# andreicuceu/vega

Hardware: AMD Instinct MI355X
Metric: model+chi2 evals/sec (Lya auto+cross) (higher is better)
Workload: dtype f64

## Files before the change

### vega_amd/csrc/vegamx.hip

```cpp
#include "vmx_device.h"
#include "vmx_fit.h"
#include "vmx_ensemble.h"
#include "vmx_nested.h"
#include "vmx_smc.h"

#include <atomic>
#include <cmath>
#include <chrono>
#include <thread>
#include <algorithm>
#include <cstdio>
#include <cstdlib>
#include <cstring>
#include <map>
#include <mutex>
#include <queue>
#include <utility>
#include <string>
#include <vector>

#ifndef VMX_MAX_LANES
#define VMX_MAX_LANES 2
#endif

// ... 73 lines not shown
    for (int i = 0; i < n; ++i) {
        for (int j = 0; j < i; ++j) out[(size_t)i * n + j] = 0.5 * (c[(size_t)i * n + j] + c[(size_t)j * n + i]);
        out[(size_t)i * n + i] = 0.5 * c[(size_t)i * n + i];
    }
    return out;
}

struct MetalHost {
    MetalDev dev{};
    DevBuf<double> mat, svec, basis, kron_a, kron_b;
    int rows = 0, cols = 0;
};

struct ItemHost {
    ItemDev dev{};
    std::vector<MetalHost*> metals;
    DevBuf<double> dm, cinv, data, vec, dist, res, z, mock_pool, add_vec;
    DevBuf<double> marg, marg_out;
    DevBuf<double> q_mat, q_w, q_lin, q_c0, q_x0, q_x, q_z;
    DevBuf<double> q_u, q_f, q_u0, q_y;
    DevBuf<double> mg_g, mg_c0, mg_y;
    DevBuf<double> mc_chol, mc_fid, q_cfull, q_m0, mc_z, mc_noise, mc_r0, mc_t;
    bool has_factor = false;
    std::vector<double> h_q_c0;
    DevBuf<int64_t> q_basis_off;
    int q_rows = 0;
    int n_templates = 0;
    int n_mocks = 0;
    DevBuf<int32_t> inv_mask;
    DevBuf<int64_t> csr_ptr; DevBuf<int32_t> csr_idx; DevBuf<double> csr_val;
    int64_t csr_nnz = 0; bool has_csr = false;
    std::vector<int32_t> mask_idx;
    bool has_dm = false, has_cinv = false, has_mask = false, has_data = false;
    bool lean_pair = false;
};

struct FitWorkspace {
    DevBuf<double> state;
    DevBuf<vmx_migrad::Spec> spec;
    DevBuf<double> base, theta, chi2;
    DevBuf<int32_t> mock_row, count, offset, done, mock, status;
    DevBuf<double> ox[vmx_migrad::MAX_STAGES], oext[vmx_migrad::MAX_STAGES], oV[vmx_migrad::MAX_STAGES], ofval[vmx_migrad::MAX_STAGES], oedm[vmx_migrad::MAX_STAGES];
    DevBuf<int32_t> oflags[vmx_migrad::MAX_STAGES], oiter[vmx_migrad::MAX_STAGES];
    DevBuf<int64_t> onfcn[vmx_migrad::MAX_STAGES];
    int32_t* pin_word = nullptr; int32_t* dpin_word = nullptr;
    hipEvent_t ev_lane = nullptr;
    std::vector<hipEvent_t> ev_gap;
    ~FitWorkspace() {
        if (pin_word) (void)hipHostFree(pin_word);
        if (ev_lane) (void)hipEventDestroy(ev_lane);
        for (auto& ev : ev_gap) (void)hipEventDestroy(ev);
    }
};
template <typename T>
static int ensure(DevBuf<T>& b, size_t count) { return b.n >= count && b.p ? 0 : b.alloc(count, false); }

struct EnsWorkspace {
    DevBuf<double> x, lnl, prop, factor, theta, chi2, fixed, lo, hi, chain, chain_lnl;
    DevBuf<int64_t> acc, n_box, n_fail;
    DevBuf<int32_t> inside, status, col;
    hipEvent_t ev_prop = nullptr, ev_lane = nullptr;
    ~EnsWorkspace() {
        if (ev_prop) (void)hipEventDestroy(ev_prop);
        if (ev_lane) (void)hipEventDestroy(ev_lane);
    }
};
// ... 551 lines not shown
    std::map<int, int64_t> odd_op_off;
    DevBuf<double> bb_basis, odd_coef, odd_op, odd_dyn, sn_a;
    int sn_n = 0; double sn_tau0 = 0.0, sn_dtau = 1.0;

    std::vector<int32_t> prior_slot;
    std::vector<double> prior_mean, prior_sigma;
    DevBuf<int32_t> d_prior_slot;
    DevBuf<double> d_prior_mean, d_prior_sigma;

    DevBuf<double> gcinv, gres, gz;
    int g_n = 0, g_ld = 0;

    int n_params = 0, max_batch = 0, model_size = 0, slab_rows = 0;
    int pad_l = 0, pad_r = 0;
    int fact_slab_rows = 0;
    std::map<int, std::vector<int>> group_splits;
    struct QuadList { DevBuf<GemmWork> work; DevBuf<int32_t> queue, nt_off; DevBuf<double> part; int n_blocks = 0; int n_entries = 0; };
    std::map<int, QuadList*> quad_lists;
    std::vector<void*> host_allocs;
    std::map<int, QuadList*> cinv_lists;
    DevBuf<double> zero_row;
    int quad_blocks = 0;
    std::vector<double> host_key, pending_key;
    bool host_key_valid = false, skip_xtab_once = false;
    bool fft_ring = true, fft_ring_attr = false;
    bool xi_sums = true;
    bool sums_dirty = true;
    std::vector<XiLeanGroup> lean_groups; std::vector<XiStaticGroup> static_groups;
    std::vector<int32_t> static_single;
    DevBuf<XiLeanGroup> d_lean_groups; DevBuf<XiStaticGroup> d_static_groups; DevBuf<ItemSums> d_item_sums;
    DevBuf<int32_t> d_static_single;
    bool sums_any = false;
    bool xi_lean = true;
    std::vector<int32_t> xi_lean_pipes, xi_rest_pipes;
    DevBuf<int32_t> d_xi_rest_pipes;
    bool ring_allowed = true;
    int last_tab_level = 0;
    bool no_tab2 = false;
    bool no_cinv_tape = false;
    bool pk_small_attr = false;
    bool kron_attr = false;
    DevBuf<double> mv_part;
    int64_t xi_total = 0, xim_total = 0;
    DevBuf<double> theta, scal, metal_bias, pl, coef, xi, xim, model, chi2;
    DevBuf<int32_t> status, mock_index, k_live, coef_win;
    DevBuf<double> pk_direct;
    bool direct = false;
    std::vector<int32_t> h_mock_index;
    int last_B = 0;
    bool last_full = false;
    bool last_taps = true;
    std::vector<double> theta_ref;
    bool quad_eligible = false, quad_mat_dirty = true, quad_lin_dirty = true, no_fuse = false;
    bool static_poly = true;
    int quad_kind = 0;
    bool quad_factored = false;
    struct MargReq { double* out; int64_t ld_out; int32_t* status; };
    const MargReq* marg_req = nullptr;
    int marg_slab_rows = 0;
    int last_form = 0;
    bool trace_host = false; double host_ns[3] = {0, 0, 0}; int64_t host_calls = 0;
    EngineDev dev{};

    double* pin_theta = nullptr; double* pin_chi2 = nullptr; int32_t* pin_status = nullptr;
    std::vector<double> blind_scale, blind_shift;
    DevBuf<double> d_blind;
// ... 992 lines not shown
        }
    }
    HIP_OK(hipStreamSynchronize(e->stream));
    HIP_OK(hipMemcpy(e->mock_index.p, e->h_mock_index.data(), (size_t)e->max_batch * sizeof(int32_t), hipMemcpyHostToDevice));
    return 0;
}

int vmx_set_global_invcov(vmx_engine* e, const double* invcov, int32_t n)
{
    REQUIRE(e && invcov && n > 0, "vmx_set_global_invcov");
    drop_lane(e);
    HIP_OK(hipSetDevice(e->device));
    const std::vector<double> half = half_form(invcov, n);
    if (e->finalized) {
        REQUIRE(e->g_n == n, "global inverse covariance size changed");
        HIP_OK(hipStreamSynchronize(e->stream));
        HIP_OK(hipMemcpy2D(e->gcinv.p, (size_t)e->g_ld * sizeof(double), half.data(), (size_t)n * sizeof(double),
                           (size_t)n * sizeof(double), n, hipMemcpyHostToDevice));
        return 0;
    }
    e->g_n = n; e->g_ld = vmx_pad(n);
    return upload_padded(e->gcinv, half.data(), n, n, e->g_ld);
}

int vmx_add_prior(vmx_engine* e, int32_t slot, double mean, double sigma)
{
    REQUIRE(e && !e->finalized && slot >= 0 && sigma != 0.0, "vmx_add_prior");
    e->prior_slot.push_back(slot); e->prior_mean.push_back(mean); e->prior_sigma.push_back(sigma);
    return 0;
}

static int poly_basis_build(vmx_engine* e);
static int xi_sum_plan(vmx_engine* e);

int vmx_finalize(vmx_engine* e, int32_t n_params, int32_t max_batch)
{
    REQUIRE(e && !e->finalized, "vmx_finalize");
    REQUIRE(n_params > 0 && max_batch > 0, "n_params / max_batch");
    REQUIRE(e->nk > 0 && !e->pipes.empty() && !e->items.empty(), "template, pipelines and items are required");
    REQUIRE(e->items.size() <= 16, "at most 16 correlation items");
    REQUIRE(e->pipes.size() * sizeof(PipeDev) <= 48 * 1024, "too many pipelines for the prologue's descriptor stage");
    for (int i = 0; i < VMX_MAX_ELL; ++i) REQUIRE(e->op_set[i], "all four FFTLog operators are required");
    HIP_OK(hipSetDevice(e->device));
    const int Bm = max_batch;
    e->n_params = n_params; e->max_batch = Bm;
    e->slab_rows = Bm > 1024 ? Bm : 1024;
    e->fact_slab_rows = std::max(1024, std::min(4 * Bm, 8192));
    if (getenv("VMX_NO_GRAPH")) e->use_graphs = false;
    if (getenv("VMX_TRACE_HOST")) e->trace_host = true;
    {
        int cus = 256;
        if (hipDeviceGetAttribute(&cus, hipDeviceAttributeMultiprocessorCount, e->device) != hipSuccess || cus <= 0) { (void)hipGetLastError(); cus = 256; }
        e->quad_blocks = 2 * cus;
    }
    if (getenv("VMX_NO_TAB2")) e->no_tab2 = true;
    if (getenv("VMX_NO_CINV_TAPE")) e->no_cinv_tape = true;
    if (getenv("VMX_NO_PK_W")) e->no_pk_w = true;
    if (getenv("VMX_NO_HOST_REDUCE")) e->no_host_reduce = true;
    if (getenv("VMX_NO_XI_LEAN")) e->xi_lean = false;
    if (getenv("VMX_NO_XI_SUMS")) e->xi_sums = false;

    auto slot_ok = [&](int s) { return s < n_params; };
    for (auto& p : e->pipes) {
        const vmx_pipe_desc& d = p.d;
        const int slots[] = {d.tracer[0].bias_slot, d.tracer[0].bias_eta_slot, d.tracer[0].beta_slot,
                             d.tracer[0].vd_sigma_slot, d.tracer[0].alpha_slot, d.tracer[1].bias_slot,
                             d.tracer[1].bias_eta_slot, d.tracer[1].beta_slot, d.tracer[1].vd_sigma_slot,
                             d.tracer[1].alpha_slot, d.growth_rate_slot, d.bias_gamma_slot, d.bias_prim_slot,
                             d.lambda_uv_slot, d.bias_gamma_e_slot, d.lambda_heii_slot, d.bias_hcd_slot,
                             d.beta_hcd_slot, d.l0_hcd_slot, d.sigma_nl_par_slot, d.sigma_nl_per_slot,
                             d.exp_par_slot, d.exp_per_slot, d.scale_slot[0], d.scale_slot[1], d.drp_slot,
                             d.croom_slot[0], d.croom_slot[1], d.mock_los_slot};
        for (int s : slots) REQUIRE(slot_ok(s), "pipeline slot exceeds n_params");
        for (int i = 0; i < 6; ++i) REQUIRE(slot_ok(d.arinyo_slot[i]), "arinyo slot exceeds n_params");
        for (int i = 0; i < d.n_smooth; ++i)
            REQUIRE(d.smooth_par_slot[i] >= 0 && d.smooth_per_slot[i] >= 0 && slot_ok(d.smooth_par_slot[i]) &&
                    slot_ok(d.smooth_per_slot[i]), "smoothing slot");
        for (int q = 0; q < 2; ++q) {
            const vmx_tracer& t = d.tracer[q];
            const int have = (t.bias_slot >= 0) + (t.bias_eta_slot >= 0) + (t.beta_slot >= 0);
            REQUIRE(have >= 2, "each tracer needs two of (bias, bias_eta, beta)");
            REQUIRE(t.evol_kind == VMX_EVOL_CROOM ? (d.croom_slot[0] >= 0 && d.croom_slot[1] >= 0) : t.alpha_slot >= 0,
                    "bias-evolution slot");
            REQUIRE(d.vd_kind == VMX_VD_NONE || !t.discrete || t.vd_sigma_slot >= 0, "velocity dispersion slot");
        }
        REQUIRE(!d.uvb || (d.bias_gamma_slot >= 0 && d.bias_prim_slot >= 0 && d.lambda_uv_slot >= 0), "UVB slots");
        REQUIRE(!d.heii || (d.bias_gamma_e_slot >= 0 && d.bias_prim_slot >= 0 && d.lambda_heii_slot >= 0), "HeII slots");
        REQUIRE(d.hcd_model == VMX_HCD_NONE || (d.bias_hcd_slot >= 0 && d.beta_hcd_slot >= 0), "HCD slots");
        REQUIRE(d.hcd_model != VMX_HCD_ROGERS || d.l0_hcd_slot >= 0, "L0_hcd slot");
        REQUIRE(d.hcd_model != VMX_HCD_FVOIGT || e->fv_n >= 2, "model-hcd = fvoigt needs vmx_set_fvoigt_table");
        REQUIRE(d.nl_model != VMX_NL_ARINYO || (d.arinyo_slot[0] >= 0 && d.arinyo_slot[2] >= 0 && d.arinyo_slot[3] >= 0 &&
                                                d.arinyo_slot[4] >= 0 && d.arinyo_slot[5] >= 0), "Arinyo slots");
        REQUIRE(!d.peak_nl || d.sigma_nl_par_slot >= 0 || d.sigma_nl_per_slot >= 0, "sigmaNL slots");
// ... 339 lines not shown
    }
    HIP_OK(hipEventCreateWithFlags(&e->ev_fork, hipEventDisableTiming));

    HIP_OK(hipHostMalloc((void**)&e->pin_theta, (size_t)Bm * n_params * sizeof(double), hipHostMallocMapped));
    HIP_OK(hipHostMalloc((void**)&e->pin_chi2, (size_t)Bm * sizeof(double), hipHostMallocMapped));
    HIP_OK(hipHostMalloc((void**)&e->pin_status, (size_t)Bm * sizeof(int32_t), hipHostMallocMapped));
    HIP_OK(hipHostMalloc((void**)&e->pin_done, sizeof(int64_t), hipHostMallocMapped));
    *e->pin_done = 0;
    if (hipHostMalloc((void**)&e->pin_part, (size_t)VMX_MAX_GROUP * 1024 * sizeof(double), hipHostMallocMapped) != hipSuccess ||
        hipHostGetDevicePointer((void**)&e->dpin_part, e->pin_part, 0) != hipSuccess) { (void)hipGetLastError(); e->dpin_part = nullptr; }
    if (getenv("VMX_NO_DONE_WORD") || hipHostGetDevicePointer((void**)&e->dpin_done, e->pin_done, 0) != hipSuccess) { (void)hipGetLastError(); e->dpin_done = nullptr; }
    if (!getenv("VMX_NO_ZERO_COPY") &&
        (hipHostGetDevicePointer((void**)&e->dpin_theta, e->pin_theta, 0) != hipSuccess ||
         hipHostGetDevicePointer((void**)&e->dpin_chi2, e->pin_chi2, 0) != hipSuccess ||
         hipHostGetDevicePointer((void**)&e->dpin_status, e->pin_status, 0) != hipSuccess)) {
        (void)hipGetLastError();
        e->dpin_theta = nullptr; e->dpin_chi2 = nullptr; e->dpin_status = nullptr;
    }

    e->quad_eligible = e->gcinv.p == nullptr && e->items.size() <= 16;
    for (auto* it : e->items) {
        int na = 0;
        if (it->dev.n_bb[VMX_BB_POST_MUL]) e->quad_eligible = false;
        for (int q = 0; q < it->dev.n_bb[VMX_BB_POST_ADD]; ++q) {
            if (it->dev.bb[VMX_BB_POST_ADD][q].func != VMX_BB_POLY) e->quad_eligible = false;
            na += it->dev.bb[VMX_BB_POST_ADD][q].n_coef;
        }
        if (na > VMX_MAX_QUAD_COEF) e->quad_eligible = false;
    }
    if (getenv("VMX_NO_QUAD")) e->quad_eligible = false;

    HIP_OK(hipStreamSynchronize(e->stream));
    e->finalized = true;
    if (poly_basis_build(e) || xi_sum_plan(e)) { e->finalized = false; return -2; }
    return 0;
}

int vmx_model_size(vmx_engine* e) { return e ? e->model_size : -1; }

int vmx_pipeline_column(vmx_engine* e, int32_t pipeline)
{
    REQUIRE(e && e->finalized && pipeline >= 0 && pipeline < (int)e->pipes.size(), "vmx_pipeline_column");
    return e->pipes[pipeline].col >= 0 ? e->pipes[pipeline].col : -3 - e->n_active;
}

constexpr double QUAD_ENTRY_STAGES = 4.0, QUAD_SKEW = 0.12;
constexpr bool QUAD_K_BANDS = true;

static vmx_engine::QuadList* quad_build_tape(vmx_engine* e, int B)
{
    const int tn = (B + GEMM_BN - 1) / GEMM_BN;
    std::vector<vmx_plan::TapeProblem> probs;
    for (auto* it : e->items) probs.push_back({it->dev.nq, it->dev.nq_pad});
    vmx_plan::Tape T = vmx_plan::plan_quad_tape(probs, tn, e->quad_blocks, QUAD_ENTRY_STAGES, QUAD_SKEW, GEMM_BM, GEMM_BK, QUAD_K_BANDS);
    auto* ql = new vmx_engine::QuadList();
    ql->n_blocks = T.n_blocks;
    ql->n_entries = (int)T.n_slots;
    if (T.work.empty()) T.work.push_back(GemmWork{-1, 0, 0, 0, 0, 0, 0, 0});
    if (ql->work.upload(T.work.data(), T.work.size()) || ql->queue.upload(T.queue.data(), T.queue.size()) ||
        ql->nt_off.upload(T.nt_off.data(), T.nt_off.size()) ||
        ql->part.alloc(std::max<size_t>((size_t)T.n_slots, 1) * 128, true)) { delete ql; return nullptr; }
    return ql;
}

static void quad_launch_list(vmx_engine* e, vmx_engine::QuadList* ql, int B)
{
    GemmGroup G{};
// ... 90 lines not shown
    if (ns == 0) return 0;
    DevBuf<double> V;
    const int64_t rows = (int64_t)ns * 3;
    if (V.alloc((size_t)VMX_MAX_ELL * rows * e->nkp, true)) return -2;
    e->cur = e->stream;
    hipLaunchKernelGGL(k_poly_basis, dim3((e->nkp + 255) / 256, ns), dim3(256), 0, e->stream, e->dev, e->d_pk_static.p, V.p);
    launch_product(e, KC_OTHER, e->op.p, e->nkp, (int64_t)e->ncp * e->nkp, e->n_coef, e->nkp,
                   V.p, e->nkp, rows * e->nkp, (int)rows, e->poly_coef.p, e->ncp, rows * e->ncp, VMX_MAX_ELL, (int)rows);
    HIP_OK(hipGetLastError());
    if (e->poly_bins_total > 0) {
        std::vector<int32_t> ok(ns, 1);
        DevBuf<int32_t> d_ok;
        if (d_ok.upload(ok.data(), ok.size())) return -2;
        int max_n = 0;
        for (int p : e->pk_static) max_n = std::max(max_n, (int)e->pipes[p].n);
        hipLaunchKernelGGL(k_poly_bins, dim3((max_n + 255) / 256, ns, 3), dim3(256), 0, e->stream, e->dev, e->d_pk_static.p,
                           e->poly_bins.p, d_ok.p);
        HIP_OK(hipGetLastError());
        HIP_OK(hipStreamSynchronize(e->stream));
        HIP_OK(hipMemcpy(ok.data(), d_ok.p, ok.size() * sizeof(int32_t), hipMemcpyDeviceToHost));
        bool changed = false;
        for (int sb = 0; sb < ns; ++sb)
            if (!ok[sb] && e->pipes[e->pk_static[sb]].poly_bins_off >= 0) { e->pipes[e->pk_static[sb]].poly_bins_off = -1; changed = true; }
        if (changed) HIP_OK(hipMemcpy(e->d_pipes.p, e->pipes.data(), e->pipes.size() * sizeof(PipeDev), hipMemcpyHostToDevice));
    }
    HIP_OK(hipStreamSynchronize(e->stream));
    for (int p : e->pk_static) (e->pipes[p].poly_bins_off >= 0 ? e->xi_static_bins : e->xi_static_taps).push_back(p);
    std::vector<int32_t> a = e->xi_static_taps, b = e->xi_static_bins;
    a.push_back(-1); b.push_back(-1);
    if (e->d_xi_static_taps.upload(a.data(), a.size()) || e->d_xi_static_bins.upload(b.data(), b.size())) return -2;
    return 0;
}

static void launch_metal_kron(vmx_engine* e, const EngineDev& D, ItemHost* it, int B)
{
    int item = 0;
    for (size_t q = 0; q < e->items.size(); ++q) if (e->items[q] == it) item = (int)q;
    size_t shmem = 0;
    for (auto* m : it->metals) {
        if (!m->dev.kron_a) continue;
        const int n = m->dev.kron_nrp * m->dev.kron_nrt;
        shmem = std::max(shmem, (size_t)(2 * n + std::max(m->dev.kron_nrp * m->dev.kron_nrp, m->dev.kron_nrt * m->dev.kron_nrt)) * sizeof(double));
    }
    if (shmem == 0) return;
    ScopedTimer t(e, KC_METAL);
    if (!e->kron_attr) { (void)hipFuncSetAttribute((const void*)k_metal_kron, hipFuncAttributeMaxDynamicSharedMemorySize, 160 * 1024); e->kron_attr = true; }
    hipLaunchKernelGGL(k_metal_kron, dim3(B, (unsigned)it->metals.size()), dim3(256), shmem, e->cur, D, item, B);
}

static bool xi_plain_args(vmx_engine* e, XiPlainArgs& A)
{
    if (e->items.size() > VMX_MAX_GROUP || e->extrapolate || e->direct) return false;
    for (size_t q = 0; q < e->items.size(); ++q) {
        const ItemHost* it = e->items[q];
        const ItemDev& d = it->dev;
        if (!it->lean_pair || d.add_vec || d.n_bb[VMX_BB_PRE_MUL] || d.n_bb[VMX_BB_PRE_ADD]) return false;
        const PipeDev& Ps = e->pipes[d.d.pipe_smooth];
        const PipeDev& Pp = e->pipes[d.d.pipe_peak];
        if (Ps.d.n_ell != Pp.d.n_ell || Ps.d.single_ell >= 0 || Pp.d.single_ell >= 0 || Ps.col < 0 || Pp.col < 0) return false;
        XiPlainItem& I = A.it[q];
        I.coord_off = Pp.coord_off; I.q_x0 = it->q_x0.p; I.q_x = it->q_x.p;
        I.n_model = d.d.n_model; I.nq = d.nq; I.nq_pad = d.nq_pad; I.pipe_s = d.d.pipe_smooth; I.pipe_p = d.d.pipe_peak;
        I.col_s = Ps.col; I.col_p = Pp.col; I.n_ell = Ps.d.n_ell; I.split_evol = Pp.split_evol; I.bao_slot = d.d.bao_amp_slot;
        I.item = (int32_t)q;
        I.radiation = Ps.d.radiation;
    }
    return true;
}

static int xi_sum_plan(vmx_engine* e)
{
    e->sums_dirty = false;
    e->lean_groups.clear(); e->static_groups.clear(); e->static_single.clear();
    e->sums_any = false;
    const int np = (int)e->pipes.size();
    struct Role { int item = -1, fkind = 0, findex = 0, metal = -1, refs = 0; bool plain = true; };
    std::vector<Role> role(np);
    int metal_base = 0;
    for (int q = 0; q < (int)e->items.size(); ++q) {
        const ItemHost* it = e->items[q];
        const vmx_item_desc& d = it->dev.d;
        auto take = [&](int p, int fkind, int findex, int metal, bool plain) {
            if (p < 0 || p >= np) return;
            Role& r = role[p];
            r.refs += 1; r.item = q; r.fkind = fkind; r.findex = findex; r.metal = metal; r.plain = r.plain && plain;
        };
        take(d.pipe_smooth, 0, 0, -1, true);
        if (d.pipe_peak != d.pipe_smooth) take(d.pipe_peak, 1, d.bao_amp_slot, -1, true);
        else role[d.pipe_smooth].plain = false;
        for (int m = 0; m < (int)it->metals.size(); ++m) {
            const MetalDev& md = it->metals[m]->dev;
            if (md.d.pipeline >= 0) take(md.d.pipeline, 2, metal_base + m, m, !md.basis && !md.svec && md.mat_off < 0 && m < 64);
        }
        metal_base += (int)it->metals.size();
    }
    std::vector<ItemSums> sums(e->items.size());
    for (size_t q = 0; q < sums.size(); ++q) { sums[q] = ItemSums{}; sums[q].n_pad = e->items[q]->dev.n_model_pad; }
    auto member_of = [&](int p) {
// ... 237 lines not shown
                if (generic) hipLaunchKernelGGL((k_pk_multipoles<KT, MS, 1, true>), grid, dim3(256), shmem, e->stream, D, gp, mp, tm, B, mu_tab_off);   \
                else hipLaunchKernelGGL((k_pk_multipoles<KT, MS, 1, false>), grid, dim3(256), shmem, e->stream, D, gp, mp, tm, B, mu_tab_off);         \
            } while (0)
            if ((int64_t)B * n_groups >= 24) VMX_LAUNCH_PK(64, 4);
            else if ((int64_t)B * n_groups >= 4) VMX_LAUNCH_PK(16, 16);
            else {
                shmem = ((size_t)e->n_rows + 2048 + (size_t)8 * e->n_rows) * sizeof(double);
                mu_tab_off = -1;
                if (!e->pk_small_attr) {
                    HIP_OK(hipFuncSetAttribute((const void*)k_pk_multipoles<8, 32, 1, true>, hipFuncAttributeMaxDynamicSharedMemorySize, (int)shmem));
                    HIP_OK(hipFuncSetAttribute((const void*)k_pk_multipoles<8, 32, 1, false>, hipFuncAttributeMaxDynamicSharedMemorySize, (int)shmem));
                    e->pk_small_attr = true;
                }
                VMX_LAUNCH_PK(8, 32);
            }
#undef VMX_LAUNCH_PK
        }
    }
    {
        const int64_t ncols = (int64_t)B * e->n_active;
        const bool pads = e->pad_l + e->pad_r > 0;
        if (ncols > 0 && pads) {
            ScopedTimer t(e, KC_FFTLOG);
            hipLaunchKernelGGL(k_pk_extrap, dim3((unsigned)(VMX_MAX_ELL * ncols)), dim3(256), 0, e->stream, D, B);
        }
        if (ncols > 0)
            launch_product(e, KC_FFTLOG, e->op.p, e->nkp, (int64_t)e->ncp * e->nkp, e->n_coef, e->nkp,
                           e->pl.p, e->nkp, ncols * e->nkp, (int)ncols, e->coef.p, e->ncp, ncols * e->ncp,
                           VMX_MAX_ELL, 0, pads ? nullptr : e->k_live.p, -1, false, e->coef_win.p);
    }
    bool xi_fused = quad && (size_t)n_pipe == 2 * e->items.size();
    for (auto* it : e->items) if (!it->metals.empty() || it->dev.d.pipe_peak == it->dev.d.pipe_smooth) xi_fused = false;
    e->last_taps = !(xi_fused && B > 8);
    if (xi_fused) {
        ScopedTimer t(e, KC_XI);
        int max_nq = 0;
        for (auto* it : e->items) max_nq = std::max(max_nq, (int)it->dev.nq_pad);
        XiPlainArgs XA{};
        if (B > 8 && xi_plain_args(e, XA))
            hipLaunchKernelGGL((D.same_grid ? k_xi_quad_plain<2, true> : k_xi_quad_plain<2, false>), dim3((max_nq + 255) / 256, (B + 1) / 2, (unsigned)e->items.size()), dim3(256), 0, e->stream, D, XA, 0, B);
        else
        hipLaunchKernelGGL(k_xi_assemble_quad, dim3((max_nq + 255) / 256, B, (unsigned)e->items.size()), dim3(256), 0, e->stream, D, 0, B <= 8 ? 1 : 0);
    } else {
        ScopedTimer t(e, KC_XI);
        int max_n = 0;
        for (auto& p : e->pipes) max_n = p.n > max_n ? p.n : max_n;
        const bool use_sums = B > 8 && !e->direct && e->xi_lean && e->xi_sums && !e->extrapolate;
        const bool sums_on = use_sums && e->sums_any && !e->sums_dirty;
        if (sums_on) { D.sums = e->d_item_sums.p; D.sums_on = 1; e->last_taps = false; }
        if (sums_on && !e->lean_groups.empty()) {
            const dim3 grid((max_n + 255) / 256, (unsigned)e->lean_groups.size(), (B + 1) / 2);
            hipLaunchKernelGGL((D.same_grid ? k_xi_bins_group<2, true> : k_xi_bins_group<2, false>), grid, dim3(256), 0, e->stream, D, e->d_lean_groups.p, B);
            if (!e->xi_rest_pipes.empty())
                hipLaunchKernelGGL(k_xi_bins<false>, dim3((max_n + 255) / 256, (unsigned)e->xi_rest_pipes.size(), B), dim3(256), 0, e->stream, D, e->d_xi_rest_pipes.p);
        } else if (B > 8 && !e->direct && !e->xi_lean_pipes.empty()) {
            XiLeanArgs LA{};
            for (size_t q = 0; q < e->xi_lean_pipes.size(); ++q) {
                const PipeDev& P = e->pipes[e->xi_lean_pipes[q]];
                XiLeanPipe& L = LA.p[q];
                L.coord_off = P.coord_off; L.xi_off = P.xi_off; L.n = P.n; L.n_pad = P.n_pad; L.pipe = e->xi_lean_pipes[q]; L.col = P.col;
                L.n_ell = P.d.n_ell; L.split_evol = P.split_evol; L.radiation = P.d.is_peak ? 0 : P.d.radiation;
            }
            const dim3 grid((max_n + 255) / 256, (unsigned)e->xi_lean_pipes.size(), (B + 1) / 2);
            hipLaunchKernelGGL((D.same_grid ? k_xi_bins_lean<2, true> : k_xi_bins_lean<2, false>), grid, dim3(256), 0, e->stream, D, LA, B);
            if (!e->xi_rest_pipes.empty())
                hipLaunchKernelGGL(k_xi_bins<false>, dim3((max_n + 255) / 256, (unsigned)e->xi_rest_pipes.size(), B), dim3(256), 0, e->stream, D, e->d_xi_rest_pipes.p);
        } else if (e->n_active > 0)
            hipLaunchKernelGGL(k_xi_bins<false>, dim3((max_n + 255) / 256, e->n_active, B), dim3(256), 0, e->stream, D, e->d_pipe_active.p);
        if (!e->pk_static.empty())
        {
            if (!e->xi_static_taps.empty())
                hipLaunchKernelGGL(k_xi_bins<true>, dim3((max_n + 255) / 256, (unsigned)e->xi_static_taps.size(), B), dim3(256), 0, e->stream, D, e->d_xi_static_taps.p);
            if (sums_on && !e->xi_static_bins.empty()) {
                if (!e->static_groups.empty()) {
// ... 1850 lines not shown
        ++e->host_calls;
    }
    return 0;
}

int64_t vmx_debug_read(vmx_engine* e, int32_t what, int32_t index, double* out, int64_t capacity)
{
    if (!e || !e->finalized || !out || e->last_B <= 0) { fail(-1, "invalid argument: vmx_debug_read"); return -1; }
    if (hipSetDevice(e->device) != hipSuccess || hipStreamSynchronize(e->stream) != hipSuccess) { fail(-2, "hip sync"); return -2; }
    wait_lane(e);
    const int B = e->last_B;
    const double* src = nullptr; int64_t count = 0;
    if (what == 0) { src = e->pl.p; count = (int64_t)VMX_MAX_ELL * B * e->n_active * e->nkp; }
    else if (what == 1) {
        if (index < 0 || index >= (int)e->pipes.size()) { fail(-1, "invalid argument: pipeline index"); return -1; }
        if (!e->last_taps) { fail(-1, "the last evaluation (chi2 only, more than 8 walkers, no metal terms) did not store the per-pipeline bins: ask for a model"); return -1; }
        src = e->xi.p + e->pipes[index].xi_off; count = (int64_t)B * e->pipes[index].n_pad;
    } else if (what == 2) { src = e->coef.p; count = (int64_t)VMX_MAX_ELL * B * e->n_active * e->ncp; }
    else if (what == 3) {
        if (index < 0 || index >= (int)e->metals.size() || e->metals[index]->dev.mat_off < 0) { fail(-1, "invalid argument: metal without matrix"); return -1; }
        int n_model_pad = 0;
        for (auto* it : e->items) for (auto* m : it->metals) if (m == e->metals[index]) n_model_pad = it->dev.n_model_pad;
        src = e->xim.p + e->metals[index]->dev.xim_off; count = (int64_t)B * n_model_pad;
    }
    else if (what == 4) {
        if (capacity < 3) { fail(-1, "invalid argument: capacity too small"); return -1; }
        int32_t live[8] = {0, 0, 0, 0, 0, 0, 0, 0};
        if (hipMemcpy(live, e->k_live.p, 8 * sizeof(int32_t), hipMemcpyDeviceToHost) != hipSuccess) { fail(-2, "hipMemcpy"); return -2; }
        out[0] = live[0]; out[1] = e->dev.k_node_max; out[2] = e->mu_lo + e->mu_hi + e->n_extra;
        if (capacity >= 4) out[3] = live[1];
        if (capacity >= 5) out[4] = e->last_tab_level;
        if (capacity >= 7) { out[5] = live[2]; out[6] = live[3]; }
        if (capacity >= 9) out[8] = e->last_form;
        if (capacity >= 8) { out[7] = live[4]; return capacity >= 9 ? 9 : 8; }
        return capacity >= 7 ? 7 : capacity >= 5 ? 5 : capacity >= 4 ? 4 : 3;
    }
    else { fail(-1, "invalid argument: what"); return -1; }
    if (count > capacity) { fail(-1, "invalid argument: capacity too small"); return -1; }
    if (hipMemcpy(out, src, (size_t)count * sizeof(double), hipMemcpyDeviceToHost) != hipSuccess) { fail(-2, "hipMemcpy"); return -2; }
    return count;
}

int vmx_matvec_device(vmx_engine* e, const double* d_A, int32_t rows, int32_t cols, const double* d_x, int32_t B,
                      double* d_y)
{
    REQUIRE(e && d_A && d_x && d_y, "vmx_matvec_device");
    wait_lane(e);
    REQUIRE(rows > 0 && cols > 0 && cols % VMX_PAD == 0, "cols (leading dimension) must be a multiple of 32, zero padded");
    REQUIRE(B > 0, "vmx_matvec_device: B > 0");
    HIP_OK(hipSetDevice(e->device));
    const int ldy = vmx_pad(rows);
    if (B <= 8) {
        launch_product(e, KC_MATVEC, d_A, cols, 0, rows, cols, d_x, cols, 0, B, d_y, ldy, 0, 1, 0);
    } else {
        const size_t need = (size_t)8 * B * ldy;
        if (e->mv_part.n < need) {
            HIP_OK(hipStreamSynchronize(e->stream));
            if (e->mv_part.alloc(need, false)) return -2;
        }
        const int ns = launch_product(e, KC_MATVEC, d_A, cols, 0, rows, cols, d_x, cols, 0, B, e->mv_part.p, ldy, 0, 1, 8 * B);
        const int64_t count = (int64_t)B * ldy;
        hipLaunchKernelGGL(k_sum_slabs, dim3((unsigned)((count + 255) / 256)), dim3(256), 0, e->cur, e->mv_part.p, d_y, count, ns);
    }
    HIP_OK(hipGetLastError());
    return 0;
}
// ... 65 lines not shown
```

### vega_amd/csrc/vmx_device.h

```cpp
#pragma once
#include <hip/hip_runtime.h>
#include <stdint.h>
#include "../../include/vegamx.h"
#include "vmx_plan.h"

#define VMX_NS 40
#define VMX_PAD 32
#define VMX_MAX_BB 32
#define VMX_MAX_METALS 64
#define VMX_MAX_QUAD_COEF 64
#define VMX_MAX_GROUP 8
#define VMX_MAX_MARG 16

enum {
    S_BIAS1 = 0, S_BB1, S_BIAS2, S_BB2,
    S_UV_BG, S_UV_BP, S_UV_LAM, S_HE_BG, S_HE_LAM,
    S_HCD_B, S_HCD_BB, S_HCD_L0,
    S_GA, S_GB, S_EA, S_EB,
    S_AQ1, S_AQ2, S_AKV, S_AAV, S_ABV, S_AKP,
    S_VD1, S_VD2,
    S_AP, S_AT, S_DRP, S_EV1A, S_EV1B, S_EV2A, S_EV2B,
    S_RAD_S, S_RAD_A, S_RAD_L, S_RAD_D, S_RAD_IL, S_RAD_ID,
    S_NO_RULE
};
// ... 3096 lines not shown
                for (int half = 0; half < 2; ++half) {
                    const double* sc = half ? scp : scs;
                    const double rrp = sc[S_AP] * (rp0 + sc[S_DRP]), rrt = sc[S_AT] * rt0;
                    const double rr2 = fma(rrp, rrp, rrt * rrt);
                    if (rr2 != 0.0) {
                        const double v = spline_legendre<false>(D, half ? Pp : Ps, b, nB, 0.5 * vmx_log(rr2), rrp * vmx_rsqrt(rr2),
                                                                0.0, 0.0, 0.0, half ? oob_p : oob_s);
                        if (half) xp = v * ev; else xs = v * ev;
                    }
                }
            }
        } else {
            xs = xi_bin_value<0>(D, it.d.pipe_smooth, b, i, nB, oob_s);
            xp = xi_bin_value<0>(D, it.d.pipe_peak, b, i, nB, oob_p);
        }
        if (oob_p || oob_s) atomicOr(&D.status[b], VMX_STATUS_BOUNDS);
        if (store_xi) {
            D.xi[Ps.xi_off + (size_t)b * Ps.n_pad + i] = xs;
            D.xi[Pp.xi_off + (size_t)b * Pp.n_pad + i] = xp;
        }
        const double bao = t[it.d.bao_amp_slot];
        v = fma(bao, xp, xs);
        if (it.add_vec) v = fma(it.add_slot >= 0 ? t[it.add_slot] : it.add_default, it.add_vec[i], v);
        if (it.n_bb[VMX_BB_PRE_MUL]) v *= bb_total(D, it, VMX_BB_PRE_MUL, t, i, it.d.n_model);
        if (it.n_bb[VMX_BB_PRE_ADD]) v += (1.0 + bao) * bb_total(D, it, VMX_BB_PRE_ADD, t, i, it.d.n_model);
        v -= it.q_x0[i];
    } else if (i < it.nq) {
        v = (1.0 + t[it.d.bao_amp_slot]) * t[it.q_slot[i - it.d.n_model]] - it.q_x0[i];
    }
    it.q_x[(size_t)b * it.nq_pad + i] = v;
}

struct XiPlainItem { int64_t coord_off; const double* q_x0; double* q_x; int32_t n_model, nq, nq_pad, pipe_s, pipe_p, col_s, col_p,
                     n_ell, split_evol, bao_slot, item, radiation; };
struct XiPlainArgs { XiPlainItem it[VMX_MAX_GROUP]; };

template <bool SAME>
__device__ __forceinline__ double xi_plain_spline(const EngineDev& D, const double* coef_col, size_t ell_stride, int n_ell, double x,
                                                  double rmu, bool& oob)
{
    const double* cf[4];
    double tt[4];
    bool on[4];
    if (SAME) {
        const bool inside = !(x < D.x0[0] || x > D.xlast[0]);
        if (!inside) oob = true;
        const double u = (x - D.x0[0]) * D.inv_h[0];
        int j = (int)floor(u);
        if (j < 0) j = 0;
        if (j > D.n_coef - 4) j = D.n_coef - 4;
        if (!(u == u)) j = 0;
        const double t = u - (double)j;
#pragma unroll
        for (int e = 0; e < 4; ++e) {
            on[e] = e < n_ell && inside;
            tt[e] = t;
            cf[e] = coef_col + (size_t)(e < n_ell ? e : 0) * ell_stride + j;
        }
    } else {
#pragma unroll
        for (int e = 0; e < 4; ++e) {
            const int ee = e < n_ell ? e : 0;
            const bool inside = !(x < D.x0[ee] || x > D.xlast[ee]);
            on[e] = e < n_ell && inside;
            if (e < n_ell && !inside) oob = true;
            const double u = (x - D.x0[ee]) * D.inv_h[ee];
            int j = (int)floor(u);
            if (j < 0) j = 0;
            if (j > D.n_coef - 4) j = D.n_coef - 4;
            if (!(u == u)) j = 0;
            tt[e] = u - (double)j;
            cf[e] = coef_col + (size_t)ee * ell_stride + j;
        }
    }
    double tap[4][4];
#pragma unroll
    for (int e = 0; e < 4; ++e)
#pragma unroll
        for (int q = 0; q < 4; ++q) tap[e][q] = cf[e][q];
    double xi = 0.0;
    const double x2 = rmu * rmu;
#pragma unroll
    for (int e = 0; e < 4; ++e) {
        const double t = tt[e], t2 = t * t, t3 = t2 * t;
        const double omt = 1.0 - t;
        const double w0 = omt * omt * omt;
        const double w1 = 3.0 * t3 - 6.0 * t2 + 4.0;
        const double w2 = -3.0 * t3 + 3.0 * t2 + 3.0 * t + 1.0;
        const double sp = (tap[e][0] * w0 + tap[e][1] * w1 + tap[e][2] * w2 + tap[e][3] * t3) * (1.0 / 6.0);
        const double leg = e == 0 ? 1.0 : e == 1 ? 0.5 * (3.0 * x2 - 1.0) : e == 2 ? 0.125 * ((35.0 * x2 - 30.0) * x2 + 3.0)
                                        : 0.0625 * (((231.0 * x2 - 315.0) * x2 + 105.0) * x2 - 5.0);
        if (on[e]) xi += sp * leg;
    }
    return xi;
}

template <int NW, bool SAME>
__global__ __launch_bounds__(256) void k_xi_quad_plain(EngineDev D, XiPlainArgs A, int item0, int B)
{
    const XiPlainItem& I = A.it[item0 + blockIdx.z];
    const int i = blockIdx.x * 256 + threadIdx.x;
    if (i >= I.nq_pad) return;
    const int b0 = blockIdx.y * NW;
    if (i >= I.n_model) {
        const ItemDev& it = D.items[I.item];
#pragma unroll
        for (int w = 0; w < NW; ++w) {
            const int b = b0 + w;
            if (b >= B) break;
            const double* t = D.theta + (size_t)b * D.n_params;
            double v = 0.0;
            if (i < I.nq) v = (1.0 + t[I.bao_slot]) * t[it.q_slot[i - I.n_model]] - I.q_x0[i];
            I.q_x[(size_t)b * I.nq_pad + i] = v;
        }
        return;
    }
    const size_t c = (size_t)I.coord_off + i;
    const double r = D.cr[c], rp0 = D.crp[c], rt0 = D.crt[c], lnz = D.clnrelz[c], growth = D.cgrowth[c], x0v = I.q_x0[i];
    const double lnz2 = I.split_evol ? D.clnrelz2[c] : 0.0;
    const size_t ncols = (size_t)B * D.n_active, ell_stride = ncols * D.ncp;
    double out[NW];
    bool oob[NW];
#pragma unroll
    for (int w = 0; w < NW; ++w) {
        const int b = min(b0 + w, B - 1);
        const double* scs = D.scal + ((size_t)b * D.n_pipe + I.pipe_s) * VMX_NS;
        const double* scp = D.scal + ((size_t)b * D.n_pipe + I.pipe_p) * VMX_NS;
        const double ev = (I.split_evol ? vmx_exp(fma(scp[S_EV1A], lnz, scp[S_EV2A] * lnz2)) : vmx_exp((scp[S_EV1A] + scp[S_EV2A]) * lnz)) * growth;
        double xs = 0.0, xp = 0.0;
        oob[w] = false;
        if (r != 0.0) {
#pragma unroll
            for (int half = 0; half < 2; ++half) {
                const double* sc = half ? scp : scs;
                const double rrp = sc[S_AP] * (rp0 + sc[S_DRP]), rrt = sc[S_AT] * rt0;
                const double rr2 = fma(rrp, rrp, rrt * rrt);
                if (rr2 != 0.0) {
                    const double* col = D.coef + ((size_t)(half ? I.col_p : I.col_s) * B + b) * D.ncp;
                    const double v = xi_plain_spline<SAME>(D, col, ell_stride, I.n_ell, 0.5 * vmx_log(rr2), rrp * vmx_rsqrt(rr2), oob[w]);
                    if (half) xp = v * ev; else xs = v * ev;
                }
            }
        }
        if (I.radiation) {
            const bool resc = I.radiation == 2;
            const double drp = scs[S_DRP];
            const double rp = resc ? fma(scs[S_AP], rp0 + drp, drp) : rp0 + drp;
            const double rtr = resc ? scs[S_AT] * rt0 : rt0;
            const double rs2 = fma(rp, rp, rtr * rtr);
            const double irs = vmx_rsqrt(rs2);
            const double rs = rs2 * irs, ms = rp * irs;
            double xr = scs[S_RAD_S] * (irs * irs) * (1.0 - scs[S_RAD_A] * (1.0 - ms * ms));
            xr *= vmx_exp(-rs * fma(1.0 + ms, scs[S_RAD_IL], scs[S_RAD_ID]));
            xs += xr;
        }
        const double bao = D.theta[(size_t)b * D.n_params + I.bao_slot];
        out[w] = fma(bao, xp, xs) - x0v;
    }
#pragma unroll
    for (int w = 0; w < NW; ++w) {
        const int b = b0 + w;
        if (b >= B) break;
        if (oob[w]) atomicOr(&D.status[b], VMX_STATUS_BOUNDS);
        I.q_x[(size_t)b * I.nq_pad + i] = out[w];
    }
}

struct XiLeanPipe { int64_t coord_off, xi_off, poly_off; int32_t n, n_pad, pipe, col, n_ell, split_evol, radiation, same_tracer; };
#define VMX_XI_LEAN_MAX 24
struct XiLeanArgs { XiLeanPipe p[VMX_XI_LEAN_MAX]; };

// ... 245 lines not shown
```

Baseline: 925,600.

## Precompute static spline weights for unit-scaled smooth component and share evolution factor

For items whose smooth pipeline has unit scaling and no drp shift, the coordinate-only work (log, rsqrt, spline knot index, cubic B-spline weights, Legendre polynomials) is computed once at finalize into a per-item table. The fused xi kernel then reuses these stored values instead of recomputing them for every batch member. It also skips recomputing the redshift-evolution exponential when adjacent batch members have identical evolution parameters. The cost is extra global memory reads of the 21-row table and some additional registers, and the precompute sets a flag to disable itself when points fall outside the spline range.

```diff
diff --git a/vega_amd/csrc/vegamx.hip b/vega_amd/csrc/vegamx.hip
--- a/vega_amd/csrc/vegamx.hip
+++ b/vega_amd/csrc/vegamx.hip
@@ -129,6 +129,7 @@
     int64_t csr_nnz = 0; bool has_csr = false;
     std::vector<int32_t> mask_idx;
     bool has_dm = false, has_cinv = false, has_mask = false, has_data = false;
+    DevBuf<double> xi_stat;
     bool lean_pair = false;
 };
 
@@ -746,6 +747,9 @@
     DevBuf<int32_t> d_static_single;
     bool sums_any = false;
     bool xi_lean = true;
+    bool xi_static_smooth = true;
+    bool xi_share_evol = true;
+    int last_static_smooth = 0;
     std::vector<int32_t> xi_lean_pipes, xi_rest_pipes;
     DevBuf<int32_t> d_xi_rest_pipes;
     bool ring_allowed = true;
@@ -1804,6 +1808,7 @@
 
 static int poly_basis_build(vmx_engine* e);
 static int xi_sum_plan(vmx_engine* e);
+static int xi_static_smooth_build(vmx_engine* e);
 
 int vmx_finalize(vmx_engine* e, int32_t n_params, int32_t max_batch)
 {
@@ -1831,6 +1836,8 @@
     if (getenv("VMX_NO_HOST_REDUCE")) e->no_host_reduce = true;
     if (getenv("VMX_NO_XI_LEAN")) e->xi_lean = false;
     if (getenv("VMX_NO_XI_SUMS")) e->xi_sums = false;
+    if (getenv("VMX_NO_STATIC_SMOOTH")) e->xi_static_smooth = false;
+    if (getenv("VMX_NO_SHARED_EVOL")) e->xi_share_evol = false;
 
     auto slot_ok = [&](int s) { return s < n_params; };
     for (auto& p : e->pipes) {
@@ -2236,7 +2243,7 @@
 
     HIP_OK(hipStreamSynchronize(e->stream));
     e->finalized = true;
-    if (poly_basis_build(e) || xi_sum_plan(e)) { e->finalized = false; return -2; }
+    if (poly_basis_build(e) || xi_sum_plan(e) || xi_static_smooth_build(e)) { e->finalized = false; return -2; }
     return 0;
 }
 
@@ -2393,6 +2400,31 @@
     return 0;
 }
 
+static int xi_static_smooth_build(vmx_engine* e)
+{
+    if (!e->xi_static_smooth || e->extrapolate || e->direct) return 0;
+    for (auto* it : e->items) {
+        const vmx_item_desc& d = it->dev.d;
+        if (d.pipe_peak == d.pipe_smooth) continue;
+        const PipeDev& Ps = e->pipes[d.pipe_smooth];
+        const PipeDev& Pp = e->pipes[d.pipe_peak];
+        if (Ps.d.scale_mode != VMX_SCALE_UNIT || Ps.d.drp_slot >= 0 || Ps.n != Pp.n || d.n_model > Pp.n || Ps.d.n_ell != Pp.d.n_ell ||
+            Ps.d.single_ell >= 0) continue;
+        const int64_t ld = vmx_pad(Pp.n);
+        if (it->xi_stat.alloc((size_t)XI_STAT_ROWS * ld, true)) return -2;
+        int32_t ok = 1;
+        DevBuf<int32_t> d_ok;
+        if (d_ok.upload(&ok, 1)) return -2;
+        hipLaunchKernelGGL(k_xi_smooth_static, dim3((Pp.n + 255) / 256), dim3(256), 0, e->stream, e->dev, Pp.coord_off, (int)Pp.n, ld,
+                           (int)Ps.d.n_ell, it->xi_stat.p, d_ok.p);
+        HIP_OK(hipGetLastError());
+        HIP_OK(hipStreamSynchronize(e->stream));
+        HIP_OK(hipMemcpy(&ok, d_ok.p, sizeof(int32_t), hipMemcpyDeviceToHost));
+        if (!ok) it->xi_stat.release();
+    }
+    return 0;
+}
+
 static void launch_metal_kron(vmx_engine* e, const EngineDev& D, ItemHost* it, int B)
 {
     int item = 0;
@@ -2425,6 +2457,7 @@
         I.col_s = Ps.col; I.col_p = Pp.col; I.n_ell = Ps.d.n_ell; I.split_evol = Pp.split_evol; I.bao_slot = d.d.bao_amp_slot;
         I.item = (int32_t)q;
         I.radiation = Ps.d.radiation;
+        I.stat_s = it->xi_stat.p; I.stat_ld = vmx_pad(Pp.n); I.share_ev = e->xi_share_evol ? 1 : 0;
     }
     return true;
 }
@@ -2728,14 +2761,16 @@
     bool xi_fused = quad && (size_t)n_pipe == 2 * e->items.size();
     for (auto* it : e->items) if (!it->metals.empty() || it->dev.d.pipe_peak == it->dev.d.pipe_smooth) xi_fused = false;
     e->last_taps = !(xi_fused && B > 8);
+    e->last_static_smooth = 0;
     if (xi_fused) {
         ScopedTimer t(e, KC_XI);
         int max_nq = 0;
         for (auto* it : e->items) max_nq = std::max(max_nq, (int)it->dev.nq_pad);
         XiPlainArgs XA{};
-        if (B > 8 && xi_plain_args(e, XA))
+        if (B > 8 && xi_plain_args(e, XA)) {
+            for (size_t q = 0; q < e->items.size(); ++q) e->last_static_smooth += XA.it[q].stat_s != nullptr;
             hipLaunchKernelGGL((D.same_grid ? k_xi_quad_plain<2, true> : k_xi_quad_plain<2, false>), dim3((max_nq + 255) / 256, (B + 1) / 2, (unsigned)e->items.size()), dim3(256), 0, e->stream, D, XA, 0, B);
-        else
+        } else
         hipLaunchKernelGGL(k_xi_assemble_quad, dim3((max_nq + 255) / 256, B, (unsigned)e->items.size()), dim3(256), 0, e->stream, D, 0, B <= 8 ? 1 : 0);
     } else {
         ScopedTimer t(e, KC_XI);
@@ -4652,6 +4687,10 @@
         if (capacity >= 5) out[4] = e->last_tab_level;
         if (capacity >= 7) { out[5] = live[2]; out[6] = live[3]; }
         if (capacity >= 9) out[8] = e->last_form;
+        if (capacity >= 10) {
+            out[9] = e->last_static_smooth; out[7] = live[4];
+            return 10;
+        }
         if (capacity >= 8) { out[7] = live[4]; return capacity >= 9 ? 9 : 8; }
         return capacity >= 7 ? 7 : capacity >= 5 ? 5 : capacity >= 4 ? 4 : 3;
     }
diff --git a/vega_amd/csrc/vmx_device.h b/vega_amd/csrc/vmx_device.h
--- a/vega_amd/csrc/vmx_device.h
+++ b/vega_amd/csrc/vmx_device.h
@@ -3152,7 +3152,9 @@
 }
 
 struct XiPlainItem { int64_t coord_off; const double* q_x0; double* q_x; int32_t n_model, nq, nq_pad, pipe_s, pipe_p, col_s, col_p,
-                     n_ell, split_evol, bao_slot, item, radiation; };
+                     n_ell, split_evol, bao_slot, item, radiation;
+                     const double* stat_s; int64_t stat_ld;
+                     int32_t share_ev, pad; };
 struct XiPlainArgs { XiPlainItem it[VMX_MAX_GROUP]; };
 
 template <bool SAME>
@@ -3215,6 +3217,82 @@
     return xi;
 }
 
+#define XI_STAT_ROWS 21
+__global__ __launch_bounds__(256) void k_xi_smooth_static(EngineDev D, int64_t coord_off, int n, int64_t ld, int n_ell, double* tab,
+                                                          int32_t* ok)
+{
+    const int i = blockIdx.x * 256 + threadIdx.x;
+    if (i >= n) return;
+    const size_t c = (size_t)coord_off + i;
+    const double r = D.cr[c], rp0 = D.crp[c], rt0 = D.crt[c];
+    uint32_t* jt = (uint32_t*)(tab + 19 * ld);
+    const double ap = 1.0, at = 1.0, drp = 0.0;
+    const double rrp = ap * (rp0 + drp), rrt = at * rt0;
+    const double rr2 = fma(rrp, rrp, rrt * rrt);
+    const bool live = r != 0.0;
+    if (live && !(rr2 != 0.0)) *ok = 0;
+    const double x = 0.5 * vmx_log(live ? rr2 : 1.0), rmu = rrp * vmx_rsqrt(live ? rr2 : 1.0);
+    const double x2 = rmu * rmu;
+#pragma unroll
+    for (int e = 0; e < 4; ++e) {
+        const int ee = e < n_ell ? e : 0;
+        const bool inside = !(x < D.x0[ee] || x > D.xlast[ee]);
+        if (live && e < n_ell && !inside) *ok = 0;
+        const double u = (x - D.x0[ee]) * D.inv_h[ee];
+        int j = (int)floor(u);
+        if (j < 0) j = 0;
+        if (j > D.n_coef - 4) j = D.n_coef - 4;
+        if (!(u == u)) j = 0;
+        const double t = u - (double)j, t2 = t * t, t3 = t2 * t;
+        const double omt = 1.0 - t;
+        const double w0 = omt * omt * omt;
+        const double w1 = 3.0 * t3 - 6.0 * t2 + 4.0;
+        const double w2 = -3.0 * t3 + 3.0 * t2 + 3.0 * t + 1.0;
+        jt[(size_t)e * ld + i] = live ? (uint32_t)j * 8u : 0u;
+        tab[(size_t)(4 * e + 0) * ld + i] = live ? w0 : 0.0;
+        tab[(size_t)(4 * e + 1) * ld + i] = live ? w1 : 0.0;
+        tab[(size_t)(4 * e + 2) * ld + i] = live ? w2 : 0.0;
+        tab[(size_t)(4 * e + 3) * ld + i] = live ? t3 : 0.0;
+        if (e > 0) {
+            const double leg = e == 1 ? 0.5 * (3.0 * x2 - 1.0) : e == 2 ? 0.125 * ((35.0 * x2 - 30.0) * x2 + 3.0)
+                                      : 0.0625 * (((231.0 * x2 - 315.0) * x2 + 105.0) * x2 - 5.0);
+            tab[(size_t)(15 + e) * ld + i] = live ? leg : 0.0;
+        }
+    }
+}
+
+struct XiStatBin { double wt[4][4], leg[4]; uint32_t joff[4]; };
+
+__device__ __forceinline__ void xi_static_load(const double* tab, size_t ld, int i, XiStatBin& S)
+{
+    const uint32_t off8 = (uint32_t)i * 8u, off4 = (uint32_t)i * 4u;
+#pragma unroll
+    for (int e = 0; e < 4; ++e) {
+        S.joff[e] = *(const uint32_t*)((const char*)(tab + 19 * ld) + (size_t)e * ld * 4 + off4);
+#pragma unroll
+        for (int q = 0; q < 4; ++q) S.wt[e][q] = *(const double*)((const char*)(tab + (size_t)(4 * e + q) * ld) + off8);
+        S.leg[e] = e == 0 ? 1.0 : *(const double*)((const char*)(tab + (size_t)(15 + e) * ld) + off8);
+    }
+}
+
+__device__ __forceinline__ double xi_static_spline(const XiStatBin& S, const double* coef_col, size_t ell_stride, int n_ell)
+{
+    double tap[4][4];
+#pragma unroll
+    for (int e = 0; e < 4; ++e) {
+        const double* cf = (const double*)((const char*)(coef_col + (size_t)(e < n_ell ? e : 0) * ell_stride) + S.joff[e]);
+#pragma unroll
+        for (int q = 0; q < 4; ++q) tap[e][q] = cf[q];
+    }
+    double xi = 0.0;
+#pragma unroll
+    for (int e = 0; e < 4; ++e) {
+        const double sp = (tap[e][0] * S.wt[e][0] + tap[e][1] * S.wt[e][1] + tap[e][2] * S.wt[e][2] + tap[e][3] * S.wt[e][3]) * (1.0 / 6.0);
+        if (e < n_ell) xi += sp * S.leg[e];
+    }
+    return xi;
+}
+
 template <int NW, bool SAME>
 __global__ __launch_bounds__(256) void k_xi_quad_plain(EngineDev D, XiPlainArgs A, int item0, int B)
 {
@@ -3241,22 +3319,36 @@
     const size_t ncols = (size_t)B * D.n_active, ell_stride = ncols * D.ncp;
     double out[NW];
     bool oob[NW];
+    double a1_prev = 0.0, a2_prev = 0.0, ev_prev = 0.0;
+    double xs_stat[NW];
+    if (I.stat_s) {
+        XiStatBin S;
+        xi_static_load(I.stat_s, (size_t)I.stat_ld, i, S);
+#pragma unroll
+        for (int w = 0; w < NW; ++w)
+            xs_stat[w] = xi_static_spline(S, D.coef + ((size_t)I.col_s * B + min(b0 + w, B - 1)) * D.ncp, ell_stride, I.n_ell);
+    }
 #pragma unroll
     for (int w = 0; w < NW; ++w) {
         const int b = min(b0 + w, B - 1);
         const double* scs = D.scal + ((size_t)b * D.n_pipe + I.pipe_s) * VMX_NS;
         const double* scp = D.scal + ((size_t)b * D.n_pipe + I.pipe_p) * VMX_NS;
-        const double ev = (I.split_evol ? vmx_exp(fma(scp[S_EV1A], lnz, scp[S_EV2A] * lnz2)) : vmx_exp((scp[S_EV1A] + scp[S_EV2A]) * lnz)) * growth;
+        const double a1 = scp[S_EV1A], a2 = scp[S_EV2A];
+        double ev;
+        if (w > 0 && I.share_ev && a1 == a1_prev && a2 == a2_prev) ev = ev_prev;
+        else ev = (I.split_evol ? vmx_exp(fma(a1, lnz, a2 * lnz2)) : vmx_exp((a1 + a2) * lnz)) * growth;
+        a1_prev = a1; a2_prev = a2; ev_prev = ev;
         double xs = 0.0, xp = 0.0;
         oob[w] = false;
         if (r != 0.0) {
 #pragma unroll
             for (int half = 0; half < 2; ++half) {
+                const double* col = D.coef + ((size_t)(half ? I.col_p : I.col_s) * B + b) * D.ncp;
+                if (half == 0 && I.stat_s) { xs = xs_stat[w] * ev; continue; }
                 const double* sc = half ? scp : scs;
                 const double rrp = sc[S_AP] * (rp0 + sc[S_DRP]), rrt = sc[S_AT] * rt0;
                 const double rr2 = fma(rrp, rrp, rrt * rrt);
                 if (rr2 != 0.0) {
-                    const double* col = D.coef + ((size_t)(half ? I.col_p : I.col_s) * B + b) * D.ncp;
                     const double v = xi_plain_spline<SAME>(D, col, ell_stride, I.n_ell, 0.5 * vmx_log(rr2), rrp * vmx_rsqrt(rr2), oob[w]);
                     if (half) xp = v * ev; else xs = v * ev;
                 }
```

Result: slower. 916,200 (-1.0%).
